# vinits5/learning3d

Measured on AMD Instinct MI355X. Metric: clouds/sec DGCNN-fwd+Chamfer B=32 N=1024; kNN HBM GB/s vs peak at 1/2/4/8 GPU, higher is better.
Workload: dtype f32 (shared-MLP GEMMs as f16x2: fp32 operands carried as an fp16 high part + an fp16 residual (unscaled between the EdgeConv kernel and conv5, 2^12-scaled elsewhere), 3 fp16 MFMA products per fp32 product, f32 accumulate, fp32-level error -- tests bound it by 2x the fp32-MFMA kernel's own error agai

## Files before the change

learning3d_amd/csrc/edgeconv_f16b.hip:

```cpp
#include <type_traits>
#include "common.h"
#include "edgeconv_layout.h"
#include "split_bf16.h"

#define EF_V2 1
#define EF_W4_BYTES ((EC_C4 / 16) * (EC_C3 / 32) * 2 * 1024)
#define EF_PAR_FLOATS (EC5_OFF_SC + 16 - EC5_OFF_W4)
#define EF_PAR_BYTES (EF_PAR_FLOATS * 4)
#define EF_LOFF_B2 (EF_W4_BYTES)
#define EF_LOFF_B3 (EF_LOFF_B2 + 4 * EC_C2)
#define EF_LOFF_B4 (EF_LOFF_B3 + 4 * EC_C3)
#define EF_LOFF_W1 (EF_LOFF_B4 + 4 * EC_C4)
#define EF_LOFF_B1 (EF_LOFF_W1 + 4 * 8 * EC_C1)
#define EF_STG_A (EF_PAR_BYTES)
#define EF_STG_B (EF_STG_A + 4 * 4096)
#define EF_LDS_BYTES (EF_STG_B + 4 * 2048)
static_assert(EC5_OFF_B2 == EC5_OFF_W4 + EF_W4_BYTES / 4 && EC5_OFF_B1 == EC5_OFF_W1 + 8 * EC_C1 && EC5_OFF_SC == EC5_OFF_B1 + EC_C1,
              "the fifth copy's tail is one contiguous run");
static_assert(EF_PAR_BYTES % 16 == 0 && EF_LDS_BYTES <= 163840, "LDS budget");
#define EF_NPL 2
#define EFO_W2 EC5_OFF_W2
#define EFO_W3 EC5_OFF_W3
#define EFO_W4 EC5_OFF_W4
#define EFO_B2 EC5_OFF_B2
#define EFO_B3 EC5_OFF_B3
#define EFO_B4 EC5_OFF_B4
#define EFO_SC EC5_OFF_SC
#define EFO_W1 EC5_OFF_W1
#define EFO_B1 EC5_OFF_B1
#define EF_KERNEL edgeconv_f16b_kernel
#define EF_ENTRY l3d_edgeconv_forward_f16b

typedef _Float16 f16x8 __attribute__((ext_vector_type(8)));
typedef uint32_t u32x4 __attribute__((ext_vector_type(4)));
struct EfBase { const char *p; };
typedef __attribute__((address_space(3))) const char *ef_lds_t;
typedef __attribute__((address_space(3))) const float *ef_ldsf_t;
typedef __attribute__((address_space(3))) char *ef_ldsw_t;
typedef EfBase ef_rsrc_t;

#define EF_ACON "a"
__device__ __forceinline__ void ef_mfma_init(f32x4 &d, const u32x4 &a, const f16x8 &b, const f32x4 &c)
{
    asm volatile("v_mfma_f32_16x16x32_f16 %0, %1, %2, %3" : "=&v"(d) : EF_ACON(a), "a"(b), "v"(c));
}
__device__ __forceinline__ void ef_mfma_acc(f32x4 &d, const u32x4 &a, const f16x8 &b)
{
    asm volatile("v_mfma_f32_16x16x32_f16 %0, %1, %2, %0" : "+v"(d) : EF_ACON(a), "a"(b));
}
__device__ __forceinline__ f16x8 ef_home_agpr(u32x4 v)
{
    f16x8 r = __builtin_bit_cast(f16x8, v);
    asm("" : "+a"(r));
    return r;
}

__device__ __forceinline__ float ef_vmax(float a, float b)
{
    float r;
    asm volatile("v_max_f32 %0, %1, %2" : "=v"(r) : "v"(a), "v"(b));
    return r;
}
__device__ __forceinline__ float ef_vmax3(float a, float b, float c)
{
    float r;
    asm volatile("v_max3_f32 %0, %1, %2, %3" : "=v"(r) : "v"(a), "v"(b), "v"(c));
    return r;
}
__device__ __forceinline__ float ef_dpp_max_x1(float give, float keep)
{
    float r;
    asm volatile("s_nop 1\n\tv_max_f32_dpp %0, %1, %2 quad_perm:[1,0,3,2] row_mask:0xf bank_mask:0xf" : "=v"(r) : "v"(give), "v"(keep));
    return r;
}
__device__ __forceinline__ float ef_dpp_max_x2(float give, float keep)
{
    float r;
    asm volatile("s_nop 1\n\tv_max_f32_dpp %0, %1, %2 quad_perm:[2,3,0,1] row_mask:0xf bank_mask:0xf" : "=v"(r) : "v"(give), "v"(keep));
    return r;
}

__device__ __forceinline__ void ef_split_pair(float a0, float a1, float c, uint32_t &h, uint32_t &m)
{
    (void)c;
    asm volatile("v_cvt_pk_f16_f32 %0, %1, %2" : "=v"(h) : "v"(a0), "v"(a1));
    asm volatile("s_nop 0\n\tv_fma_mixlo_f16 %0, %1, 1.0, -%2 op_sel_hi:[0,0,1]" : "=v"(m) : "v"(a0), "v"(h));
    asm volatile("v_fma_mixhi_f16 %0, %1, 1.0, -%2 op_sel:[0,0,1] op_sel_hi:[0,0,1]" : "+v"(m) : "v"(a1), "v"(h));
}

struct EfLane {
    bool odd, hi;
    unsigned laneoff;
    ef_rsrc_t rs;
    ef_lds_t w4lds;
    float *prow;
    ef_ldsw_t stgA, stgB;
    float mres;
    size_t bn;
};

struct EfScale {
    float split, pool;
};

struct EfTmp {
    f32x4 mx[2];
    u32x4 qh, qm;
    f32x2 xs[2];
};

template <int MT, bool LAST> struct EfN { static constexpr int UNITS = LAST ? 12 : 6 * MT + 12; };

template <int MT, bool LAST, bool RAW, bool PLANES, int U>
__device__ __forceinline__ void ef_micro(f32x4 (&h)[2][MT], f16x8 (&pl)[2][MT], EfTmp &T, int ch0, const EfLane &L, const EfScale &sc, float &ovf)
{
    const float c = sc.split;
    constexpr int NT = LAST ? 0 : 6 * MT;
    if constexpr (U < NT) {
        constexpr int t = U / 6, k = U % 6;
        if constexpr (k < 2) {
#pragma unroll
            for (int r = 0; r < 4; r++) h[k][t][r] = RAW ? ef_vmax(h[k][t][r], 0.f) : fmaxf(h[k][t][r], 0.f);
        } else {
            constexpr int i = k - 2;
            uint32_t a, b;
            ef_split_pair(h[i >> 1][t][2 * (i & 1)], h[i >> 1][t][2 * (i & 1) + 1], c, a, b);
            T.qh[i] = a;
            T.qm[i] = b;
            if constexpr (i == 3) {
                pl[0][t] = ef_home_agpr(T.qh);
                pl[1][t] = ef_home_agpr(T.qm);
            }
        }
    } else if constexpr (U < NT + 8) {
        constexpr int k = (U - NT) / 4, r = (U - NT) % 4;
        static_assert(MT >= 3 && MT <= 5, "row tiles per wave");
        if constexpr (RAW) {
            float m = ef_vmax3(h[k][0][r], h[k][1][r], h[k][2][r]);
            if constexpr (MT == 4) m = ef_vmax(m, h[k][3][r]);
            if constexpr (MT == 5) m = ef_vmax3(m, h[k][3][r], h[k][4][r]);
            T.mx[k][r] = m;
        } else {
            float m = h[k][0][r];
#pragma unroll
            for (int t = 1; t < MT; t++) m = fmaxf(m, h[k][t][r]);
            T.mx[k][r] = m;
        }
    } else {
        constexpr int k = (U - NT - 8) / 2, part = (U - NT - 8) % 2;
        if constexpr (part == 0) {
            const float k0 = L.odd ? T.mx[k][2] : T.mx[k][0], g0 = L.odd ? T.mx[k][0] : T.mx[k][2];
            const float k1 = L.odd ? T.mx[k][3] : T.mx[k][1], g1 = L.odd ? T.mx[k][1] : T.mx[k][3];
            T.xs[k][0] = ef_dpp_max_x1(g0, k0);
            T.xs[k][1] = ef_dpp_max_x1(g1, k1);
        } else {
            const float kk = L.hi ? T.xs[k][1] : T.xs[k][0], gg = L.hi ? T.xs[k][0] : T.xs[k][1];
            float v = ef_dpp_max_x2(gg, kk);
            if constexpr (LAST) v = ef_vmax(v, 0.f);
            if constexpr (!LAST) ovf = ef_vmax(ovf, v * sc.split);
            v *= sc.pool;
            if constexpr (PLANES) {
                ovf = ef_vmax(ovf, v);
                const _Float16 hh = (_Float16)v;
                const _Float16 mm = (_Float16)((v - (float)hh) * L.mres);
                typedef __attribute__((address_space(3))) _Float16 *lh_t;
                if constexpr (!LAST) {
                    const int off = ((ch0 + 16 * k) >> 3) * 64;
                    *(lh_t)(L.stgA + off) = hh;
                    *(lh_t)(L.stgA + off + 2048) = mm;
                } else {
                    const int m = (ch0 - (EC_C1 + EC_C2 + EC_C3)) >> 5;
                    const int off = ((m >> 1) & 1) * 1024 + (m & 1) * 512 + (2 * k) * 64;
                    *(lh_t)(L.stgB + off) = hh;
                    *(lh_t)(L.stgB + off + 256) = mm;
                }
            } else {
                L.prow[ch0 + 16 * k] = v;
            }
        }
    }
}

template <int I0, int I1, class F>
__device__ __forceinline__ void ef_static_for(F &&f)
{
    if constexpr (I0 < I1) {
        f(std::integral_constant<int, I0>{});
        ef_static_for<I0 + 1, I1>(f);
    }
}

template <int MT, bool LAST, bool RAW, bool PLANES>
__device__ __forceinline__ void ef_finish_all(f32x4 (&h)[2][MT], f16x8 (&pl)[2][MT], int ch0, const EfLane &L, const EfScale &sc, float &ovf)
{
    EfTmp T;
    ef_static_for<0, EfN<MT, LAST>::UNITS>([&](auto u) { ef_micro<MT, LAST, RAW, PLANES, decltype(u)::value>(h, pl, T, ch0, L, sc, ovf); });
}

#define EF_PIN() asm volatile("" ::: "memory")

#ifndef EF_PD
#define EF_PD 4
#endif
struct EfRing {
    u32x4 a[EF_PD][EF_NPL];
    f32x4 bv[2];
};
struct EfNext {
    int woff;
    ef_ldsf_t bias;
    int mp;
    int steps;
};

__device__ __forceinline__ u32x4 ef_ldfrag(ef_rsrc_t rs, int byte_off, int frag, unsigned laneoff)
{
    return *(const u32x4 *)(rs.p + (size_t)byte_off + (size_t)frag * 1024 + laneoff);
}

__device__ __forceinline__ u32x4 ef_ldfrag_lds(ef_lds_t base, int frag, unsigned laneoff)
{
    return *(__attribute__((address_space(3))) const u32x4 *)(base + frag * 1024 + laneoff);
}

__device__ __forceinline__ void ef_ring_fill(EfRing &R, ef_rsrc_t rs, int woff, ef_ldsf_t bias4g, int mp, int steps, int lane)
{
#pragma unroll
    for (int d = 0; d < EF_PD; d++)
#pragma unroll
        for (int p = 0; p < EF_NPL; p++) R.a[d][p] = ef_ldfrag(rs, woff, (mp * steps + d) * EF_NPL + p, (unsigned)lane * 16u);
    R.bv[0] = *(__attribute__((address_space(3))) const f32x4 *)(bias4g + 32 * mp);
    R.bv[1] = *(__attribute__((address_space(3))) const f32x4 *)(bias4g + 32 * mp + 16);
}

template <int MT, int S, bool PREV_LAST, bool PREV_RAW, bool PLANES, int NSL, bool OWN_LDS = false, bool NX_LDS = false>
__device__ __forceinline__ void ef_pair(int mp, const EfNext &nx, const f16x8 (&pin)[S][2][MT], const f16x8 (&pin_last)[2][MT],
                                        int woff, EfRing &R,
                                        f32x4 (&acc)[2][MT], f32x4 (&hp)[2][MT], f16x8 (&po_prev)[2][MT],
                                        int ch_prev, const EfLane &L, const EfScale &c_prev, float &ovf)
{
    static_assert(2 * S >= EF_PD, "a pair is at least EF_PD steps long");
    constexpr int NU = EfN<MT, PREV_LAST>::UNITS;
    EfTmp T;
    ef_static_for<0, 2 * S>([&](auto rc) {
        constexpr int r = decltype(rc)::value, s = r >> 1, mm = r & 1;
        u32x4 an[EF_NPL];
        if constexpr (r + EF_PD < 2 * S) {
#pragma unroll
            for (int p = 0; p < EF_NPL; p++)
                an[p] = OWN_LDS ? ef_ldfrag_lds(L.w4lds, (mp * 2 * S + r + EF_PD) * EF_NPL + p, L.laneoff)
                                : ef_ldfrag(L.rs, woff, (mp * 2 * S + r + EF_PD) * EF_NPL + p, L.laneoff);
        } else {
#pragma unroll
            for (int p = 0; p < EF_NPL; p++)
                an[p] = NX_LDS ? ef_ldfrag_lds(L.w4lds, (nx.mp * nx.steps + (r + EF_PD - 2 * S)) * EF_NPL + p, L.laneoff)
                               : ef_ldfrag(L.rs, nx.woff, (nx.mp * nx.steps + (r + EF_PD - 2 * S)) * EF_NPL + p, L.laneoff);
        }
        EF_PIN();
        if constexpr (s == S - 1 && mm == 0 && NSL < 2 * S * 3 * MT)
            asm volatile("s_nop 7");
        ef_static_for<0, 3>([&](auto pc) {
            constexpr int prod = decltype(pc)::value;
            constexpr int pa = prod == 0 ? 1 : 0;
            constexpr int pb = prod == 1 ? 1 : 0;
            ef_static_for<0, MT>([&](auto tc) {
                constexpr int t = decltype(tc)::value;
                const f16x8 &bop = s == S - 1 ? pin_last[pb][t] : pin[s][pb][t];
                if constexpr (s == 0 && prod == 0) ef_mfma_init(acc[mm][t], R.a[0][pa], bop, R.bv[mm]);
                else ef_mfma_acc(acc[mm][t], R.a[0][pa], bop);
                constexpr int slot = (r * 3 + prod) * MT + t;
                if constexpr (slot < NSL)
                    ef_static_for<slot * NU / NSL, (slot + 1) * NU / NSL>([&](auto u) {
                        ef_micro<MT, PREV_LAST, PREV_RAW, PLANES, decltype(u)::value>(hp, po_prev, T, ch_prev, L, c_prev, ovf);
                    });
            });
        });
        if constexpr (r == 1) {
            R.bv[0] = *(__attribute__((address_space(3))) const f32x4 *)(nx.bias + 32 * nx.mp);
            R.bv[1] = *(__attribute__((address_space(3))) const f32x4 *)(nx.bias + 32 * nx.mp + 16);
            EF_PIN();
        }
#pragma unroll
        for (int p = 0; p < EF_NPL; p++) {
#pragma unroll
            for (int d = 0; d + 1 < EF_PD; d++) R.a[d][p] = R.a[d + 1][p];
            R.a[EF_PD - 1][p] = an[p];
        }
    });
}

struct EfNoHook { template <class I> __device__ __forceinline__ void operator()(I) const {} };

template <int MT, int S, int NPAIR, bool LAST, bool UNROLL, bool IN_RAW, bool PLANES, class HOOK = EfNoHook, bool OWN_LDS = false, bool AFTER_LDS = false>
__device__ __forceinline__ void ef_layer(const f16x8 (&pin)[S][2][MT], f16x8 (&pout)[LAST ? 1 : NPAIR][2][MT],
                                         int woff, ef_ldsf_t bias4g, const EfNext &after, EfRing &R, int ch_own,
                                         f32x4 (&accA)[2][MT], f32x4 (&accB)[2][MT], int ch_in,
                                         int *mp_out, const EfLane &L, int rot, const EfScale &c_in, const EfScale &c_own, float &ovf,
                                         HOOK &&hook = EfNoHook())
{
    static_assert(NPAIR % 2 == 0 && S >= 2, "pairs are processed two at a time; deferred finish needs S >= 2");
    constexpr int NS = 2 * S * 3 * MT, NSD = (S - 1) * 6 * MT;
    f16x8 last[2][MT];
    auto in_layer = [&](int mp) { return EfNext{woff, bias4g, mp, 2 * S}; };
    if constexpr (UNROLL) {
        static_assert(NPAIR == 2 || NPAIR == 4, "unrolled layers have 2 or 4 output pairs");
        static_assert(!OWN_LDS, "only the rolled (last) layer keeps its weights in LDS");
        ef_pair<MT, S, false, IN_RAW, PLANES, NSD>(0, in_layer(1), pin, last, woff, R, accA, accB, last, ch_in, L, c_in, ovf);
        if constexpr (NPAIR > 2)
            ef_pair<MT, S, LAST, true, PLANES, NS>(1, in_layer(2), pin, last, woff, R, accB, accA, pout[0], ch_own, L, c_own, ovf);
        else
            ef_pair<MT, S, LAST, true, PLANES, NS, false, AFTER_LDS>(1, after, pin, last, woff, R, accB, accA, pout[0], ch_own, L, c_own, ovf);
        if constexpr (NPAIR == 4) {
            ef_pair<MT, S, LAST, true, PLANES, NS>(2, in_layer(3), pin, last, woff, R, accA, accB, pout[1], ch_own + 32, L, c_own, ovf);
            ef_pair<MT, S, LAST, true, PLANES, NS, false, AFTER_LDS>(3, after, pin, last, woff, R, accB, accA, pout[2], ch_own + 64, L, c_own, ovf);
        }
        *mp_out = NPAIR - 1;
    } else {
        (void)rot;
        ef_pair<MT, S, false, IN_RAW, PLANES, NSD, OWN_LDS, OWN_LDS>(0, in_layer(1), pin, last, woff, R, accA, accB, last, ch_in, L, c_in, ovf);
        ef_static_for<1, NPAIR>([&](auto ic) {
            constexpr int i = decltype(ic)::value;
            hook(ic);
            constexpr bool more = i + 1 < NPAIR;
            const EfNext nx = more ? in_layer(i + 1) : after;
            if constexpr (i & 1)
                ef_pair<MT, S, LAST, true, PLANES, NS, OWN_LDS, more ? OWN_LDS : AFTER_LDS>(i, nx, pin, last, woff, R, accB, accA, pout[0],
                                                                                          ch_own + 32 * (i - 1), L, c_own, ovf);
            else
                ef_pair<MT, S, LAST, true, PLANES, NS, OWN_LDS, more ? OWN_LDS : AFTER_LDS>(i, nx, pin, last, woff, R, accA, accB, pout[0],
                                                                                          ch_own + 32 * (i - 1), L, c_own, ovf);
        });
        *mp_out = NPAIR - 1;
    }
}


template <int MT>
struct EfGather {
    int nb[MT];
    float c;
    float b1[MT];
    int b, nc;
};

template <int MT>
__device__ __forceinline__ void ef_gather_idx(EfGather<MT> &G, int tile, int tiles_per_cloud, int N, int k, const float *__restrict__ xyz,
                                              const int64_t *__restrict__ idx, int wave, int j, int g)
{
    const int b = tile / tiles_per_cloud, xb = tile - b * tiles_per_cloud;
    const int n = (xb * 4 + wave) * 4 + (j >> 2);
    const int nc = min(n, N - 1);
    G.b = b;
    G.nc = nc;
    const float *cloud = xyz + (size_t)b * N * 3;
    G.c = cloud[nc * 3 + (g == 0 ? 1 : 2)];
    const int64_t *row = idx + (size_t)b * N * k;
#pragma unroll
    for (int t = 0; t < MT; t++) {
        const int jj = 4 * t + (j & 3);
        G.nb[t] = (int)row[nc * k + (jj < k ? jj : 0)];
    }
}

template <int MT>
__device__ __forceinline__ void ef_gather_xyz(EfGather<MT> &G, int N, const float *__restrict__ xyz, int g)
{
    const float *cloud = xyz + (size_t)G.b * N * 3;
    const int comp = g < 3 ? g : 0;
#pragma unroll
    for (int t = 0; t < MT; t++) {
        int r = g < 3 ? G.nb[t] : G.nc;
        asm("" : "+v"(r));
        G.b1[t] = cloud[r * 3 + comp];
    }
}

template <int MT, bool PLANES>
__global__ __launch_bounds__(256, 1) void EF_KERNEL(const float *__restrict__ xyz,
                                                              const int64_t *__restrict__ idx, int B, int N, int k,
                                                              const float *packed,
                                                              float *__restrict__ pooled,
                                                              int *__restrict__ range_flag, float mres)
{
#define EF_T(i)
    EF_T(0);
    constexpr int CTOT = EC_C1 + EC_C2 + EC_C3 + EC_C4;
    const int lane = threadIdx.x & 63, wave = threadIdx.x >> 6;
    const int j = lane & 15, g = lane >> 4;
    const int tiles_per_cloud = (N + 15) / 16, ntiles = B * tiles_per_cloud;
    EfLane L;
    L.laneoff = (unsigned)lane * 16u;
    L.rs.p = (const char *)packed;
    L.odd = j & 1;
    L.hi = j & 2;
    const int cl = 4 * g + ((j & 1) * 2 + ((j >> 1) & 1));
    L.bn = (size_t)B * N;
    L.mres = mres;
    extern __shared__ __attribute__((aligned(16))) unsigned char ef_lds[];
    L.w4lds = (ef_lds_t)ef_lds;
    {
        const int cell = (cl >> 3) * 64 + (j >> 2) * 16 + (cl & 7) * 2;
        L.stgA = (ef_ldsw_t)ef_lds + EF_STG_A + wave * 4096 + cell;
        L.stgB = (ef_ldsw_t)ef_lds + EF_STG_B + wave * 2048 + cell;
    }
    typedef __attribute__((address_space(3))) const u32x4 *ef_ldsq_t;
    const ef_ldsq_t rdA = (ef_ldsq_t)((ef_lds_t)ef_lds + EF_STG_A + wave * 4096 + lane * 16);
    const ef_ldsq_t rdB = (ef_ldsq_t)((ef_lds_t)ef_lds + EF_STG_B + wave * 2048 + lane * 16);
    if (PLANES && blockIdx.x == 0 && threadIdx.x == 0)
        *(float *)((_Float16 *)pooled + 2 * 512 * L.bn) = packed[EFO_SC + 12];
    const int po = PLANES ? 8 : 4;
    const EfScale s1 = {packed[EFO_SC + 0], packed[EFO_SC + po + 0]}, s2 = {packed[EFO_SC + 1], packed[EFO_SC + po + 1]},
                  s3 = {packed[EFO_SC + 2], packed[EFO_SC + po + 2]}, s4 = {1.0f, packed[EFO_SC + po + 3]};
    float ovf = 0.f;
    constexpr int w2 = EFO_W2 * 4, w3 = EFO_W3 * 4, w4 = EFO_W4 * 4;
    const ef_ldsf_t bs2 = (ef_ldsf_t)((ef_lds_t)ef_lds + EF_LOFF_B2) + 4 * g, bs3 = (ef_ldsf_t)((ef_lds_t)ef_lds + EF_LOFF_B3) + 4 * g,
                    bs4 = (ef_ldsf_t)((ef_lds_t)ef_lds + EF_LOFF_B4) + 4 * g;

    int tile = blockIdx.x;
    EfGather<MT> G;
    ef_gather_idx<MT>(G, tile, tiles_per_cloud, N, k, xyz, idx, wave, j, g);
    EF_PIN();
    ef_gather_xyz<MT>(G, N, xyz, g);
    EF_PIN();
    {
        typedef const __attribute__((address_space(1))) void *gp_t;
        typedef __attribute__((address_space(3))) void *lp_t;
        constexpr int NCH = EF_PAR_BYTES / 1024;
        const char *src = (const char *)(packed + EFO_W4);
#pragma unroll
        for (int c = 0; c < (NCH + 3) / 4; c++) {
            const int ch = c * 4 + wave;
            if (ch < NCH) __builtin_amdgcn_global_load_lds((gp_t)(src + ch * 1024 + lane * 16), (lp_t)(ef_lds + ch * 1024), 16, 0, 0);
        }
        EF_PIN();
        constexpr int REM = EF_PAR_BYTES - NCH * 1024;
        static_assert(REM % 16 == 0 && REM < 1024, "remainder in 16-byte pieces");
        if (threadIdx.x < REM / 16) ((uint4 *)(ef_lds + NCH * 1024))[threadIdx.x] = ((const uint4 *)(src + NCH * 1024))[threadIdx.x];
    }
    asm volatile("s_waitcnt vmcnt(0)" ::: "memory");
    __syncthreads();
    EfRing R;
    ef_ring_fill(R, L.rs, EFO_W2 * 4, bs2, 0, 2 * (EC_C1 / 32), lane);
    EF_PIN();
#pragma unroll
    for (int t = 0; t < MT; t++) asm volatile("" : "+v"(G.b1[t]));
    asm volatile("" : "+v"(G.c));

    for (; tile < ntiles; tile += gridDim.x) {
    const int b = G.b;
    L.prow = pooled + ((size_t)b * N + G.nc) * CTOT + cl;
    const int n_st = min(((tile - b * tiles_per_cloud) * 4 + wave) * 4 + (lane & 3), N - 1);
    char *const img_pt = (char *)pooled + ((size_t)b * N + n_st) * 16;
    const size_t row_bytes = L.bn * 16;
    float b1[MT][2];
#pragma unroll
    for (int t = 0; t < MT; t++) { b1[t][0] = G.b1[t]; b1[t][1] = g < 2 ? G.c : 0.f; }
    const int tile_next = tile + (int)gridDim.x;
    const bool has_next = tile_next < ntiles;

    EF_T(1);
    f16x8 p1[EC_C1 / 32][2][MT];
    f32x4 accA[2][MT], accB[2][MT];
    {
        typedef __attribute__((address_space(3))) const f32x2 *lw1_t;
        typedef __attribute__((address_space(3))) const f32x4 *lb1_t;
        const lw1_t w1 = (lw1_t)((ef_lds_t)ef_lds + EF_LOFF_W1);
        const ef_ldsf_t b1p = (ef_ldsf_t)((ef_lds_t)ef_lds + EF_LOFF_B1) + 4 * g;
        f32x2 a1[EC_C1 / 16];
        f32x4 bv1[EC_C1 / 16];
#pragma unroll
        for (int m = 0; m < EC_C1 / 16; m++) { a1[m] = w1[m * 64 + lane]; bv1[m] = *(lb1_t)(b1p + 16 * m); }
        static_assert(EC_C1 == 64, "layer 1 is two M-tile pairs");
        auto mfma1 = [&](f32x4 &d, float a, float b, const f32x4 &c, bool first) {
            if (first) asm volatile("v_mfma_f32_16x16x4_f32 %0, %1, %2, %3" : "=&v"(d) : "v"(a), "v"(b), "v"(c));
            else asm volatile("v_mfma_f32_16x16x4_f32 %0, %1, %2, %0" : "+v"(d) : "v"(a), "v"(b));
        };
#pragma unroll
        for (int t = 0; t < MT; t++) asm volatile("" ::"v"(b1[t][0]), "v"(b1[t][1]));
        asm volatile("s_nop 3");
#pragma unroll
        for (int mm = 0; mm < 2; mm++)
#pragma unroll
            for (int s = 0; s < 2; s++)
#pragma unroll
                for (int t = 0; t < MT; t++) mfma1(accA[mm][t], a1[mm][s], b1[t][s], bv1[mm], s == 0);
        constexpr int NU1 = EfN<MT, false>::UNITS, NSL1 = 4 * MT;
        EfTmp T1;
        ef_static_for<0, NSL1>([&](auto sc) {
            constexpr int slot = decltype(sc)::value, mm = slot / (2 * MT), s = (slot / MT) % 2, t = slot % MT;
            mfma1(accB[mm][t], a1[2 + mm][s], b1[t][s], bv1[2 + mm], s == 0);
            ef_static_for<slot * NU1 / NSL1, (slot + 1) * NU1 / NSL1>([&](auto u) {
                ef_micro<MT, false, true, PLANES, decltype(u)::value>(accA, p1[0], T1, 0, L, s1, ovf);
            });
        });
#pragma unroll
        for (int m = 0; m < EC_C1 / 16; m++) asm volatile("" ::"v"(bv1[m]), "v"(a1[m]));
    }
    int mp_last;

    EF_T(2);
    f16x8 p2[EC_C2 / 32][2][MT];
    ef_layer<MT, EC_C1 / 32, EC_C2 / 32, false, true, true, PLANES>(
        p1, p2, w2, bs2, EfNext{w3, bs3, 0, 2 * (EC_C2 / 32)}, R, EC_C1, accA, accB,
        32 * (EC_C1 / 32 - 1), &mp_last, L, 0, s1, s2, ovf);
    EF_T(3);
    f16x8 p3[EC_C3 / 32][2][MT];
    ef_layer<MT, EC_C2 / 32, EC_C3 / 32, false, true, true, PLANES, EfNoHook, false, true>(
        p2, p3, w3, bs3, EfNext{w4, bs4, 0, 2 * (EC_C3 / 32)}, R, EC_C1 + EC_C2, accA, accB,
        EC_C1 + 32 * (EC_C2 / 32 - 1), &mp_last, L, 0, s2, s3, ovf);
    EF_T(4);
    f16x8 dummy[1][2][MT];
    u32x4 X;
#define EF_ST16(ptr, val) (*(u32x4 *)(ptr) = (val))
    auto st_a = [&](int c) { EF_ST16(img_pt + (size_t)((c >> 1) * 64 + (c & 1) * 16 + (lane >> 2)) * row_bytes, X); EF_PIN(); };
    auto st_b = [&](int m0) {
        const int row = ((lane >> 4) & 1) * 64 + (EC_C1 + EC_C2 + EC_C3) / 8 + 4 * (m0 + (lane >> 5)) + ((lane >> 2) & 3);
        EF_ST16(img_pt + (size_t)row * row_bytes, X);
        EF_PIN();
    };
    auto hook = [&](auto ic) {
        constexpr int i = decltype(ic)::value;
        if constexpr (PLANES) {
            if constexpr (i >= 2 && i <= 5) st_a(i - 2);
            if constexpr (i == 6) st_b(0);
            if constexpr (i == 7) st_b(2);
            if constexpr (i >= 1 && i <= 4) X = rdA[(i - 1) * 64];
            if constexpr (i == 5 || i == 7) X = rdB[0];
            if constexpr (i == 6) X = rdB[64];
            EF_PIN();
        }
        if (has_next) {
            if constexpr (i == 2) { ef_gather_idx<MT>(G, tile_next, tiles_per_cloud, N, k, xyz, idx, wave, j, g); EF_PIN(); }
            if constexpr (i == 6) { ef_gather_xyz<MT>(G, N, xyz, g); EF_PIN(); }
            if constexpr (i == 7) {
#pragma unroll
                for (int t = 0; t < MT; t++) asm volatile("" : "+v"(G.b1[t]));
                asm volatile("" : "+v"(G.c));
            }
        }
    };
    ef_layer<MT, EC_C3 / 32, EC_C4 / 32, true, false, true, PLANES, decltype(hook) &, true, false>(
        p3, dummy, w4, bs4, EfNext{w2, bs2, 0, 2 * (EC_C1 / 32)}, R, EC_C1 + EC_C2 + EC_C3, accA, accB,
        EC_C1 + EC_C2 + 32 * (EC_C3 / 32 - 1), &mp_last, L, 0, s3, s4, ovf, hook);
    if constexpr (PLANES) st_b(4);
    asm volatile("s_nop 15\n\ts_nop 15");
    ef_finish_all<MT, true, true, PLANES>(accB, dummy[0], EC_C1 + EC_C2 + EC_C3 + 32 * mp_last, L, s4, ovf);
    if constexpr (PLANES) { X = rdB[64]; st_b(6); }
    EF_T(5);
    }
    if (!(ovf <= 60000.f) && range_flag) *(volatile int *)range_flag = 1;
}

static int ef_grid(int ntiles)
{
    static thread_local int cus[16] = {0};
    int dev = 0;
    if (hipGetDevice(&dev) != hipSuccess || dev < 0 || dev >= 16) dev = 0;
    if (cus[dev] == 0) {
        int n = 0;
        if (hipDeviceGetAttribute(&n, hipDeviceAttributeMultiprocessorCount, dev) != hipSuccess || n <= 0) n = 256;
        cus[dev] = n;
    }
    return ntiles < cus[dev] ? ntiles : cus[dev];
}

extern "C" int EF_ENTRY(const float *xyz, const int64_t *idx, int B, int N, int k,
                                        const float *packed, void *out, int out_mode, int *range_flag, l3d_stream_t stream)
{
    L3D_REQUIRE(xyz && idx && packed && out && B > 0 && N > 0 && k > 0 && out_mode >= 0 && out_mode <= 2);
    const float mres = out_mode == 2 ? 1.0f : 4096.0f;
    if (k > 20 || B > 65535 || (((size_t)packed) & 15) || (((size_t)out) & 15)) return L3D_ERR_UNSUPPORTED;
    const long ntiles = (long)B * l3d_divup(N, 16);
    if (ntiles > 0x7fffffffL / 2) return L3D_ERR_UNSUPPORTED;
    dim3 grid(ef_grid((int)ntiles)), block(256);
    hipStream_t st = (hipStream_t)stream;
    float *o = (float *)out;
    const size_t lds = EF_LDS_BYTES;
    if (out_mode == 0) {
        if (k <= 16) hipLaunchKernelGGL((EF_KERNEL<4, false>), grid, block, lds, st, xyz, idx, B, N, k, packed, o, range_flag, mres);
        else              hipLaunchKernelGGL((EF_KERNEL<5, false>), grid, block, lds, st, xyz, idx, B, N, k, packed, o, range_flag, mres);
    } else {
        if (k <= 16) hipLaunchKernelGGL((EF_KERNEL<4, true>), grid, block, lds, st, xyz, idx, B, N, k, packed, o, range_flag, mres);
        else              hipLaunchKernelGGL((EF_KERNEL<5, true>), grid, block, lds, st, xyz, idx, B, N, k, packed, o, range_flag, mres);
    }
    return l3d_check_launch();
}
```

Before: 118,100.

## Defer pooled-channel plane split into later layer and rebalance epilogue interleave

Pooled max results for the first three layers are now kept in AGPRs and converted to fp16 hi/residual planes later, during the last layer's MFMA steps, through a staged unpark hook. Before this, the split and LDS stores ran right after each layer. The quad-reduction and split helpers are merged into multi-instruction asm blocks that use SGPR lane masks with v_cndmask instead of per-lane bools. Epilogue micro-units are now spread over MFMA slots by weighted cost rather than uniformly. The aim is to hide VALU epilogue work under matrix ops. The cost is higher AGPR pressure and a fragile compile-time schedule.

```diff
diff --git a/learning3d_amd/csrc/edgeconv_f16b.hip b/learning3d_amd/csrc/edgeconv_f16b.hip
--- a/learning3d_amd/csrc/edgeconv_f16b.hip
+++ b/learning3d_amd/csrc/edgeconv_f16b.hip
@@ -61,35 +61,87 @@
     asm volatile("v_max_f32 %0, %1, %2" : "=v"(r) : "v"(a), "v"(b));
     return r;
 }
-__device__ __forceinline__ float ef_vmax3(float a, float b, float c)
+
+template <int MT>
+__device__ __forceinline__ float ef_pool_rows(float a0, float a1, float a2, float a3, float a4)
 {
     float r;
-    asm volatile("v_max3_f32 %0, %1, %2, %3" : "=v"(r) : "v"(a), "v"(b), "v"(c));
+    if constexpr (MT == 3) asm volatile("v_max3_f32 %0, %1, %2, %3" : "=v"(r) : "v"(a0), "v"(a1), "v"(a2));
+    if constexpr (MT == 4) asm volatile("v_max3_f32 %0, %1, %2, %3\n\tv_max_f32 %0, %0, %4" : "=&v"(r) : "v"(a0), "v"(a1), "v"(a2), "v"(a3));
+    if constexpr (MT == 5)
+        asm volatile("v_max3_f32 %0, %1, %2, %3\n\tv_max3_f32 %0, %0, %4, %5" : "=&v"(r) : "v"(a0), "v"(a1), "v"(a2), "v"(a3), "v"(a4));
     return r;
 }
-__device__ __forceinline__ float ef_dpp_max_x1(float give, float keep)
-{
-    float r;
-    asm volatile("s_nop 1\n\tv_max_f32_dpp %0, %1, %2 quad_perm:[1,0,3,2] row_mask:0xf bank_mask:0xf" : "=v"(r) : "v"(give), "v"(keep));
-    return r;
-}
-__device__ __forceinline__ float ef_dpp_max_x2(float give, float keep)
-{
-    float r;
-    asm volatile("s_nop 1\n\tv_max_f32_dpp %0, %1, %2 quad_perm:[2,3,0,1] row_mask:0xf bank_mask:0xf" : "=v"(r) : "v"(give), "v"(keep));
-    return r;
-}
-
-__device__ __forceinline__ void ef_split_pair(float a0, float a1, float c, uint32_t &h, uint32_t &m)
-{
-    (void)c;
-    asm volatile("v_cvt_pk_f16_f32 %0, %1, %2" : "=v"(h) : "v"(a0), "v"(a1));
-    asm volatile("s_nop 0\n\tv_fma_mixlo_f16 %0, %1, 1.0, -%2 op_sel_hi:[0,0,1]" : "=v"(m) : "v"(a0), "v"(h));
-    asm volatile("v_fma_mixhi_f16 %0, %1, 1.0, -%2 op_sel:[0,0,1] op_sel_hi:[0,0,1]" : "+v"(m) : "v"(a1), "v"(h));
+
+__device__ __forceinline__ void ef_quad_step1(const f32x4 &a, const f32x4 &b, uint64_t odd, f32x2 &xa, f32x2 &xb)
+{
+    float k0, g0, k1, g1, k2, g2, k3, g3, r0, r1, r2, r3;
+    asm volatile("v_cndmask_b32 %[k0], %[a0], %[a2], %[odd]\n\t"
+                 "v_cndmask_b32 %[g0], %[a2], %[a0], %[odd]\n\t"
+                 "v_cndmask_b32 %[k1], %[a1], %[a3], %[odd]\n\t"
+                 "v_cndmask_b32 %[g1], %[a3], %[a1], %[odd]\n\t"
+                 "v_cndmask_b32 %[k2], %[b0], %[b2], %[odd]\n\t"
+                 "v_cndmask_b32 %[g2], %[b2], %[b0], %[odd]\n\t"
+                 "v_cndmask_b32 %[k3], %[b1], %[b3], %[odd]\n\t"
+                 "v_cndmask_b32 %[g3], %[b3], %[b1], %[odd]\n\t"
+                 "v_max_f32_dpp %[r0], %[g0], %[k0] quad_perm:[1,0,3,2] row_mask:0xf bank_mask:0xf\n\t"
+                 "v_max_f32_dpp %[r1], %[g1], %[k1] quad_perm:[1,0,3,2] row_mask:0xf bank_mask:0xf\n\t"
+                 "v_max_f32_dpp %[r2], %[g2], %[k2] quad_perm:[1,0,3,2] row_mask:0xf bank_mask:0xf\n\t"
+                 "v_max_f32_dpp %[r3], %[g3], %[k3] quad_perm:[1,0,3,2] row_mask:0xf bank_mask:0xf"
+                 : [k0] "=&v"(k0), [g0] "=&v"(g0), [k1] "=&v"(k1), [g1] "=&v"(g1), [k2] "=&v"(k2), [g2] "=&v"(g2), [k3] "=&v"(k3),
+                   [g3] "=&v"(g3), [r0] "=&v"(r0), [r1] "=&v"(r1), [r2] "=&v"(r2), [r3] "=&v"(r3)
+                 : [a0] "v"(a[0]), [a1] "v"(a[1]), [a2] "v"(a[2]), [a3] "v"(a[3]), [b0] "v"(b[0]), [b1] "v"(b[1]), [b2] "v"(b[2]),
+                   [b3] "v"(b[3]), [odd] "s"(odd));
+    xa[0] = r0; xa[1] = r1; xb[0] = r2; xb[1] = r3;
+}
+
+template <bool LAST>
+__device__ __forceinline__ void ef_quad_step2(const f32x2 &xa, const f32x2 &xb, uint64_t hi, float split, float &va, float &vb, float &ovf)
+{
+    float k0, g0, k1, g1, t0, t1;
+    if constexpr (LAST) {
+        (void)split; (void)t0; (void)t1; (void)ovf;
+        asm volatile("v_cndmask_b32 %[k0], %[a0], %[a1], %[hi]\n\t"
+                     "v_cndmask_b32 %[g0], %[a1], %[a0], %[hi]\n\t"
+                     "v_cndmask_b32 %[k1], %[b0], %[b1], %[hi]\n\t"
+                     "v_cndmask_b32 %[g1], %[b1], %[b0], %[hi]\n\t"
+                     "v_max_f32_dpp %[va], %[g0], %[k0] quad_perm:[2,3,0,1] row_mask:0xf bank_mask:0xf\n\t"
+                     "v_max_f32_e64 %[va], %[va], 0\n\t"
+                     "v_max_f32_dpp %[vb], %[g1], %[k1] quad_perm:[2,3,0,1] row_mask:0xf bank_mask:0xf\n\t"
+                     "v_max_f32_e64 %[vb], %[vb], 0"
+                     : [k0] "=&v"(k0), [g0] "=&v"(g0), [k1] "=&v"(k1), [g1] "=&v"(g1), [va] "=&v"(va), [vb] "=&v"(vb)
+                     : [a0] "v"(xa[0]), [a1] "v"(xa[1]), [b0] "v"(xb[0]), [b1] "v"(xb[1]), [hi] "s"(hi));
+    } else {
+        asm volatile("v_cndmask_b32 %[k0], %[a0], %[a1], %[hi]\n\t"
+                     "v_cndmask_b32 %[g0], %[a1], %[a0], %[hi]\n\t"
+                     "v_cndmask_b32 %[k1], %[b0], %[b1], %[hi]\n\t"
+                     "v_cndmask_b32 %[g1], %[b1], %[b0], %[hi]\n\t"
+                     "v_max_f32_dpp %[va], %[g0], %[k0] quad_perm:[2,3,0,1] row_mask:0xf bank_mask:0xf\n\t"
+                     "v_mul_f32 %[t0], %[va], %[sp]\n\t"
+                     "v_max_f32_dpp %[vb], %[g1], %[k1] quad_perm:[2,3,0,1] row_mask:0xf bank_mask:0xf\n\t"
+                     "v_mul_f32 %[t1], %[vb], %[sp]\n\t"
+                     "v_max_f32 %[ovf], %[ovf], %[t0]\n\t"
+                     "v_max_f32 %[ovf], %[ovf], %[t1]"
+                     : [k0] "=&v"(k0), [g0] "=&v"(g0), [k1] "=&v"(k1), [g1] "=&v"(g1), [va] "=&v"(va), [vb] "=&v"(vb), [t0] "=&v"(t0),
+                       [t1] "=&v"(t1), [ovf] "+v"(ovf)
+                     : [a0] "v"(xa[0]), [a1] "v"(xa[1]), [b0] "v"(xb[0]), [b1] "v"(xb[1]), [hi] "s"(hi), [sp] "v"(split));
+    }
+}
+
+__device__ __forceinline__ void ef_split_2pairs(float a0, float a1, float b0, float b1, uint32_t &ha, uint32_t &ma, uint32_t &hb, uint32_t &mb)
+{
+    asm volatile("v_cvt_pk_f16_f32 %0, %4, %5\n\t"
+                 "v_cvt_pk_f16_f32 %2, %6, %7\n\t"
+                 "v_fma_mixlo_f16 %1, %4, 1.0, -%0 op_sel_hi:[0,0,1]\n\t"
+                 "v_fma_mixlo_f16 %3, %6, 1.0, -%2 op_sel_hi:[0,0,1]\n\t"
+                 "v_fma_mixhi_f16 %1, %5, 1.0, -%0 op_sel:[0,0,1] op_sel_hi:[0,0,1]\n\t"
+                 "v_fma_mixhi_f16 %3, %7, 1.0, -%2 op_sel:[0,0,1] op_sel_hi:[0,0,1]"
+                 : "=&v"(ha), "=&v"(ma), "=&v"(hb), "=&v"(mb)
+                 : "v"(a0), "v"(a1), "v"(b0), "v"(b1));
 }
 
 struct EfLane {
-    bool odd, hi;
+    uint64_t odd, hi;
     unsigned laneoff;
     ef_rsrc_t rs;
     ef_lds_t w4lds;
@@ -103,31 +155,71 @@
     float split, pool;
 };
 
+struct EfOut {
+    float ovf;
+    float park[(EC_C1 + EC_C2 + EC_C3) / 16];
+    float last[2];
+};
+
+struct EfStage {
+    float v, t;
+    uint32_t h, m;
+};
+template <int G, bool PARKED>
+__device__ __forceinline__ void ef_unpark(EfStage &s, float parked, float pool, float mres, float &ovf, ef_ldsw_t cell)
+{
+    typedef __attribute__((address_space(3))) _Float16 *lh_t;
+    if constexpr (G == 0 && PARKED) asm volatile("v_accvgpr_read_b32 %0, %1\n\tv_mul_f32 %0, %2, %0" : "=&v"(s.v) : "a"(parked), "s"(pool));
+    if constexpr (G == 0 && !PARKED) asm volatile("v_mul_f32 %0, %2, %1" : "=v"(s.v) : "v"(parked), "s"(pool));
+    if constexpr (G == 1) asm volatile("v_max_f32 %0, %0, %2\n\tv_cvt_f16_f32 %1, %2" : "+v"(ovf), "=&v"(s.h) : "v"(s.v));
+    if constexpr (G == 2) asm volatile("v_cvt_f32_f16 %0, %1\n\tv_sub_f32 %0, %2, %0" : "=&v"(s.t) : "v"(s.h), "v"(s.v));
+    if constexpr (G == 3) asm volatile("v_mul_f32 %0, %2, %1\n\tv_cvt_f16_f32 %0, %0" : "=&v"(s.m) : "v"(s.t), "s"(mres));
+    if constexpr (G == 4) {
+        *(lh_t)cell = __builtin_bit_cast(_Float16, (uint16_t)s.h);
+        *(lh_t)(cell + (PARKED ? 2048 : 256)) = __builtin_bit_cast(_Float16, (uint16_t)s.m);
+    }
+}
+
 struct EfTmp {
     f32x4 mx[2];
     u32x4 qh, qm;
     f32x2 xs[2];
 };
 
-template <int MT, bool LAST> struct EfN { static constexpr int UNITS = LAST ? 12 : 6 * MT + 12; };
+template <int MT, bool LAST> struct EfN {
+    static constexpr int NT = LAST ? 0 : 6 * MT;
+    static constexpr int UNITS = NT + 10;
+    static constexpr int weight(int u) { return u < NT ? (u % 6 < 4 ? 2 : 8) : u < NT + 8 ? 2 : u == NT + 8 ? 12 : LAST ? 20 : 12; }
+    static constexpr int first(int u0, int u1, int n, int s)
+    {
+        int W = 0, cum = 0;
+        for (int u = u0; u < u1; u++) W += weight(u);
+        for (int u = u0; u < u1; u++) {
+            if (cum * n / W >= s) return u;
+            cum += weight(u);
+        }
+        return u1;
+    }
+};
 
 template <int MT, bool LAST, bool RAW, bool PLANES, int U>
-__device__ __forceinline__ void ef_micro(f32x4 (&h)[2][MT], f16x8 (&pl)[2][MT], EfTmp &T, int ch0, const EfLane &L, const EfScale &sc, float &ovf)
-{
-    const float c = sc.split;
-    constexpr int NT = LAST ? 0 : 6 * MT;
+__device__ __forceinline__ void ef_micro(f32x4 (&h)[2][MT], f16x8 (&pl)[2][MT], EfTmp &T, int ch0, const EfLane &L, const EfScale &sc, EfOut &O)
+{
+    constexpr int NT = EfN<MT, LAST>::NT;
     if constexpr (U < NT) {
         constexpr int t = U / 6, k = U % 6;
-        if constexpr (k < 2) {
-#pragma unroll
-            for (int r = 0; r < 4; r++) h[k][t][r] = RAW ? ef_vmax(h[k][t][r], 0.f) : fmaxf(h[k][t][r], 0.f);
+        if constexpr (k < 4) {
+#pragma unroll
+            for (int r = 2 * (k & 1); r < 2 * (k & 1) + 2; r++) h[k >> 1][t][r] = RAW ? ef_vmax(h[k >> 1][t][r], 0.f) : fmaxf(h[k >> 1][t][r], 0.f);
         } else {
-            constexpr int i = k - 2;
-            uint32_t a, b;
-            ef_split_pair(h[i >> 1][t][2 * (i & 1)], h[i >> 1][t][2 * (i & 1) + 1], c, a, b);
-            T.qh[i] = a;
-            T.qm[i] = b;
-            if constexpr (i == 3) {
+            constexpr int m = k - 4;
+            uint32_t ha, ma, hb, mb;
+            ef_split_2pairs(h[m][t][0], h[m][t][1], h[m][t][2], h[m][t][3], ha, ma, hb, mb);
+            T.qh[2 * m] = ha;
+            T.qm[2 * m] = ma;
+            T.qh[2 * m + 1] = hb;
+            T.qm[2 * m + 1] = mb;
+            if constexpr (m == 1) {
                 pl[0][t] = ef_home_agpr(T.qh);
                 pl[1][t] = ef_home_agpr(T.qm);
             }
@@ -136,46 +228,28 @@
         constexpr int k = (U - NT) / 4, r = (U - NT) % 4;
         static_assert(MT >= 3 && MT <= 5, "row tiles per wave");
         if constexpr (RAW) {
-            float m = ef_vmax3(h[k][0][r], h[k][1][r], h[k][2][r]);
-            if constexpr (MT == 4) m = ef_vmax(m, h[k][3][r]);
-            if constexpr (MT == 5) m = ef_vmax3(m, h[k][3][r], h[k][4][r]);
-            T.mx[k][r] = m;
+            T.mx[k][r] = ef_pool_rows<MT>(h[k][0][r], h[k][1][r], h[k][2][r], h[k][MT > 3 ? 3 : 0][r], h[k][MT > 4 ? 4 : 0][r]);
         } else {
             float m = h[k][0][r];
 #pragma unroll
             for (int t = 1; t < MT; t++) m = fmaxf(m, h[k][t][r]);
             T.mx[k][r] = m;
         }
+    } else if constexpr (U == NT + 8) {
+        ef_quad_step1(T.mx[0], T.mx[1], L.odd, T.xs[0], T.xs[1]);
     } else {
-        constexpr int k = (U - NT - 8) / 2, part = (U - NT - 8) % 2;
-        if constexpr (part == 0) {
-            const float k0 = L.odd ? T.mx[k][2] : T.mx[k][0], g0 = L.odd ? T.mx[k][0] : T.mx[k][2];
-            const float k1 = L.odd ? T.mx[k][3] : T.mx[k][1], g1 = L.odd ? T.mx[k][1] : T.mx[k][3];
-            T.xs[k][0] = ef_dpp_max_x1(g0, k0);
-            T.xs[k][1] = ef_dpp_max_x1(g1, k1);
-        } else {
-            const float kk = L.hi ? T.xs[k][1] : T.xs[k][0], gg = L.hi ? T.xs[k][0] : T.xs[k][1];
-            float v = ef_dpp_max_x2(gg, kk);
-            if constexpr (LAST) v = ef_vmax(v, 0.f);
-            if constexpr (!LAST) ovf = ef_vmax(ovf, v * sc.split);
-            v *= sc.pool;
-            if constexpr (PLANES) {
-                ovf = ef_vmax(ovf, v);
-                const _Float16 hh = (_Float16)v;
-                const _Float16 mm = (_Float16)((v - (float)hh) * L.mres);
-                typedef __attribute__((address_space(3))) _Float16 *lh_t;
-                if constexpr (!LAST) {
-                    const int off = ((ch0 + 16 * k) >> 3) * 64;
-                    *(lh_t)(L.stgA + off) = hh;
-                    *(lh_t)(L.stgA + off + 2048) = mm;
-                } else {
-                    const int m = (ch0 - (EC_C1 + EC_C2 + EC_C3)) >> 5;
-                    const int off = ((m >> 1) & 1) * 1024 + (m & 1) * 512 + (2 * k) * 64;
-                    *(lh_t)(L.stgB + off) = hh;
-                    *(lh_t)(L.stgB + off + 256) = mm;
-                }
+        float vk[2];
+        ef_quad_step2<LAST>(T.xs[0], T.xs[1], L.hi, sc.split, vk[0], vk[1], O.ovf);
+#pragma unroll
+        for (int k = 0; k < 2; k++) {
+            if constexpr (PLANES && !LAST) {
+                float p = vk[k];
+                asm("" : "+a"(p));
+                O.park[(ch0 >> 4) + k] = p;
+            } else if constexpr (PLANES) {
+                O.last[k] = vk[k];
             } else {
-                L.prow[ch0 + 16 * k] = v;
+                L.prow[ch0 + 16 * k] = vk[k] * sc.pool;
             }
         }
     }
@@ -190,11 +264,25 @@
     }
 }
 
+template <int G>
+__device__ __forceinline__ void ef_last_stage(EfStage &s, EfOut &O, int k, int ch0, const EfLane &L, const EfScale &sc)
+{
+    const int m = (ch0 - (EC_C1 + EC_C2 + EC_C3)) >> 5;
+    ef_unpark<G, false>(s, O.last[k], sc.pool, L.mres, O.ovf, L.stgB + ((m >> 1) & 1) * 1024 + (m & 1) * 512 + (2 * k) * 64);
+}
+
 template <int MT, bool LAST, bool RAW, bool PLANES>
-__device__ __forceinline__ void ef_finish_all(f32x4 (&h)[2][MT], f16x8 (&pl)[2][MT], int ch0, const EfLane &L, const EfScale &sc, float &ovf)
+__device__ __forceinline__ void ef_finish_all(f32x4 (&h)[2][MT], f16x8 (&pl)[2][MT], int ch0, const EfLane &L, const EfScale &sc, EfOut &O)
 {
     EfTmp T;
-    ef_static_for<0, EfN<MT, LAST>::UNITS>([&](auto u) { ef_micro<MT, LAST, RAW, PLANES, decltype(u)::value>(h, pl, T, ch0, L, sc, ovf); });
+    ef_static_for<0, EfN<MT, LAST>::UNITS>([&](auto u) { ef_micro<MT, LAST, RAW, PLANES, decltype(u)::value>(h, pl, T, ch0, L, sc, O); });
+    if constexpr (LAST && PLANES) {
+        EfStage s[2];
+        ef_static_for<0, 5>([&](auto g) {
+            ef_last_stage<decltype(g)::value>(s[0], O, 0, ch0, L, sc);
+            ef_last_stage<decltype(g)::value>(s[1], O, 1, ch0, L, sc);
+        });
+    }
 }
 
 #define EF_PIN() asm volatile("" ::: "memory")
@@ -233,14 +321,23 @@
     R.bv[1] = *(__attribute__((address_space(3))) const f32x4 *)(bias4g + 32 * mp + 16);
 }
 
-template <int MT, int S, bool PREV_LAST, bool PREV_RAW, bool PLANES, int NSL, bool OWN_LDS = false, bool NX_LDS = false>
+struct EfNoHook { template <class... I> __device__ __forceinline__ void operator()(I...) const {} };
+
+template <int MT, int S, bool PREV_LAST, bool PREV_RAW, bool PLANES, int NSL, bool OWN_LDS = false, bool NX_LDS = false, class EXTRA = EfNoHook>
 __device__ __forceinline__ void ef_pair(int mp, const EfNext &nx, const f16x8 (&pin)[S][2][MT], const f16x8 (&pin_last)[2][MT],
                                         int woff, EfRing &R,
                                         f32x4 (&acc)[2][MT], f32x4 (&hp)[2][MT], f16x8 (&po_prev)[2][MT],
-                                        int ch_prev, const EfLane &L, const EfScale &c_prev, float &ovf)
+                                        int ch_prev, const EfLane &L, const EfScale &c_prev, EfOut &O, EXTRA &&extra = EfNoHook())
 {
     static_assert(2 * S >= EF_PD, "a pair is at least EF_PD steps long");
-    constexpr int NU = EfN<MT, PREV_LAST>::UNITS;
+    typedef EfN<MT, PREV_LAST> E;
+    constexpr int NU = E::UNITS, NS = 2 * S * 3 * MT;
+    constexpr int NA = NSL < NS ? E::NT : NU;
+    constexpr bool WAYOUT = PREV_LAST && PLANES;
+    constexpr int NSU = WAYOUT ? (2 * S - 5) * 3 * MT : NSL;
+    static_assert(!WAYOUT || (2 * S > 5 && NSL == NS), "five steps for the way out");
+    EfStage TS[2];
+    static_assert(NSL == NS || !PREV_LAST, "a deferred finish is the finish of a layer that has planes");
     EfTmp T;
     ef_static_for<0, 2 * S>([&](auto rc) {
         constexpr int r = decltype(rc)::value, s = r >> 1, mm = r & 1;
@@ -269,10 +366,14 @@
                 if constexpr (s == 0 && prod == 0) ef_mfma_init(acc[mm][t], R.a[0][pa], bop, R.bv[mm]);
                 else ef_mfma_acc(acc[mm][t], R.a[0][pa], bop);
                 constexpr int slot = (r * 3 + prod) * MT + t;
-                if constexpr (slot < NSL)
-                    ef_static_for<slot * NU / NSL, (slot + 1) * NU / NSL>([&](auto u) {
-                        ef_micro<MT, PREV_LAST, PREV_RAW, PLANES, decltype(u)::value>(hp, po_prev, T, ch_prev, L, c_prev, ovf);
-                    });
+                constexpr int ub = slot < NSU ? E::first(0, NA, NSU, slot) : WAYOUT ? NU : E::first(NA, NU, NS - NSL, slot - NSL);
+                constexpr int ue = slot < NSU ? E::first(0, NA, NSU, slot + 1) : WAYOUT ? NU : E::first(NA, NU, NS - NSL, slot + 1 - NSL);
+                ef_static_for<ub, ue>([&](auto u) {
+                    ef_micro<MT, PREV_LAST, PREV_RAW, PLANES, decltype(u)::value>(hp, po_prev, T, ch_prev, L, c_prev, O);
+                });
+                if constexpr (WAYOUT && slot >= NSU && (slot % (3 * MT) == 5 || slot % (3 * MT) == 10))
+                    ef_last_stage<(slot - NSU) / (3 * MT)>(TS[slot % (3 * MT) == 10], O, slot % (3 * MT) == 10, ch_prev, L, c_prev);
+                extra(std::integral_constant<int, slot>{});
             });
         });
         if constexpr (r == 1) {
@@ -289,14 +390,14 @@
     });
 }
 
-struct EfNoHook { template <class I> __device__ __forceinline__ void operator()(I) const {} };
-
-template <int MT, int S, int NPAIR, bool LAST, bool UNROLL, bool IN_RAW, bool PLANES, class HOOK = EfNoHook, bool OWN_LDS = false, bool AFTER_LDS = false>
+
+template <int MT, int S, int NPAIR, bool LAST, bool UNROLL, bool IN_RAW, bool PLANES, class HOOK = EfNoHook, bool OWN_LDS = false, bool AFTER_LDS = false,
+          class EXTRA = EfNoHook>
 __device__ __forceinline__ void ef_layer(const f16x8 (&pin)[S][2][MT], f16x8 (&pout)[LAST ? 1 : NPAIR][2][MT],
                                          int woff, ef_ldsf_t bias4g, const EfNext &after, EfRing &R, int ch_own,
                                          f32x4 (&accA)[2][MT], f32x4 (&accB)[2][MT], int ch_in,
-                                         int *mp_out, const EfLane &L, int rot, const EfScale &c_in, const EfScale &c_own, float &ovf,
-                                         HOOK &&hook = EfNoHook())
+                                         int *mp_out, const EfLane &L, int rot, const EfScale &c_in, const EfScale &c_own, EfOut &O,
+                                         HOOK &&hook = EfNoHook(), EXTRA &&extra = EfNoHook())
 {
     static_assert(NPAIR % 2 == 0 && S >= 2, "pairs are processed two at a time; deferred finish needs S >= 2");
     constexpr int NS = 2 * S * 3 * MT, NSD = (S - 1) * 6 * MT;
@@ -305,30 +406,31 @@
     if constexpr (UNROLL) {
         static_assert(NPAIR == 2 || NPAIR == 4, "unrolled layers have 2 or 4 output pairs");
         static_assert(!OWN_LDS, "only the rolled (last) layer keeps its weights in LDS");
-        ef_pair<MT, S, false, IN_RAW, PLANES, NSD>(0, in_layer(1), pin, last, woff, R, accA, accB, last, ch_in, L, c_in, ovf);
+        ef_pair<MT, S, false, IN_RAW, PLANES, NSD>(0, in_layer(1), pin, last, woff, R, accA, accB, last, ch_in, L, c_in, O);
         if constexpr (NPAIR > 2)
-            ef_pair<MT, S, LAST, true, PLANES, NS>(1, in_layer(2), pin, last, woff, R, accB, accA, pout[0], ch_own, L, c_own, ovf);
+            ef_pair<MT, S, LAST, true, PLANES, NS>(1, in_layer(2), pin, last, woff, R, accB, accA, pout[0], ch_own, L, c_own, O);
         else
-            ef_pair<MT, S, LAST, true, PLANES, NS, false, AFTER_LDS>(1, after, pin, last, woff, R, accB, accA, pout[0], ch_own, L, c_own, ovf);
+            ef_pair<MT, S, LAST, true, PLANES, NS, false, AFTER_LDS>(1, after, pin, last, woff, R, accB, accA, pout[0], ch_own, L, c_own, O);
         if constexpr (NPAIR == 4) {
-            ef_pair<MT, S, LAST, true, PLANES, NS>(2, in_layer(3), pin, last, woff, R, accA, accB, pout[1], ch_own + 32, L, c_own, ovf);
-            ef_pair<MT, S, LAST, true, PLANES, NS, false, AFTER_LDS>(3, after, pin, last, woff, R, accB, accA, pout[2], ch_own + 64, L, c_own, ovf);
+            ef_pair<MT, S, LAST, true, PLANES, NS>(2, in_layer(3), pin, last, woff, R, accA, accB, pout[1], ch_own + 32, L, c_own, O);
+            ef_pair<MT, S, LAST, true, PLANES, NS, false, AFTER_LDS>(3, after, pin, last, woff, R, accB, accA, pout[2], ch_own + 64, L, c_own, O);
         }
         *mp_out = NPAIR - 1;
     } else {
         (void)rot;
-        ef_pair<MT, S, false, IN_RAW, PLANES, NSD, OWN_LDS, OWN_LDS>(0, in_layer(1), pin, last, woff, R, accA, accB, last, ch_in, L, c_in, ovf);
+        ef_pair<MT, S, false, IN_RAW, PLANES, NSD, OWN_LDS, OWN_LDS>(0, in_layer(1), pin, last, woff, R, accA, accB, last, ch_in, L, c_in, O);
         ef_static_for<1, NPAIR>([&](auto ic) {
             constexpr int i = decltype(ic)::value;
             hook(ic);
             constexpr bool more = i + 1 < NPAIR;
             const EfNext nx = more ? in_layer(i + 1) : after;
+            auto ex = [&](auto sc) { extra(ic, sc); };
             if constexpr (i & 1)
-                ef_pair<MT, S, LAST, true, PLANES, NS, OWN_LDS, more ? OWN_LDS : AFTER_LDS>(i, nx, pin, last, woff, R, accB, accA, pout[0],
-                                                                                          ch_own + 32 * (i - 1), L, c_own, ovf);
+                ef_pair<MT, S, LAST, true, PLANES, NS, OWN_LDS, more ? OWN_LDS : AFTER_LDS, decltype(ex) &>(i, nx, pin, last, woff, R, accB, accA, pout[0],
+                                                                                                           ch_own + 32 * (i - 1), L, c_own, O, ex);
             else
-                ef_pair<MT, S, LAST, true, PLANES, NS, OWN_LDS, more ? OWN_LDS : AFTER_LDS>(i, nx, pin, last, woff, R, accA, accB, pout[0],
-                                                                                          ch_own + 32 * (i - 1), L, c_own, ovf);
+                ef_pair<MT, S, LAST, true, PLANES, NS, OWN_LDS, more ? OWN_LDS : AFTER_LDS, decltype(ex) &>(i, nx, pin, last, woff, R, accA, accB, pout[0],
+                                                                                                           ch_own + 32 * (i - 1), L, c_own, O, ex);
         });
         *mp_out = NPAIR - 1;
     }
@@ -391,8 +493,8 @@
     EfLane L;
     L.laneoff = (unsigned)lane * 16u;
     L.rs.p = (const char *)packed;
-    L.odd = j & 1;
-    L.hi = j & 2;
+    L.odd = __ballot(j & 1);
+    L.hi = __ballot(j & 2);
     const int cl = 4 * g + ((j & 1) * 2 + ((j >> 1) & 1));
     L.bn = (size_t)B * N;
     L.mres = mres;
@@ -411,7 +513,8 @@
     const int po = PLANES ? 8 : 4;
     const EfScale s1 = {packed[EFO_SC + 0], packed[EFO_SC + po + 0]}, s2 = {packed[EFO_SC + 1], packed[EFO_SC + po + 1]},
                   s3 = {packed[EFO_SC + 2], packed[EFO_SC + po + 2]}, s4 = {1.0f, packed[EFO_SC + po + 3]};
-    float ovf = 0.f;
+    EfOut O;
+    O.ovf = 0.f;
     constexpr int w2 = EFO_W2 * 4, w3 = EFO_W3 * 4, w4 = EFO_W4 * 4;
     const ef_ldsf_t bs2 = (ef_ldsf_t)((ef_lds_t)ef_lds + EF_LOFF_B2) + 4 * g, bs3 = (ef_ldsf_t)((ef_lds_t)ef_lds + EF_LOFF_B3) + 4 * g,
                     bs4 = (ef_ldsf_t)((ef_lds_t)ef_lds + EF_LOFF_B4) + 4 * g;
@@ -489,8 +592,8 @@
         ef_static_for<0, NSL1>([&](auto sc) {
             constexpr int slot = decltype(sc)::value, mm = slot / (2 * MT), s = (slot / MT) % 2, t = slot % MT;
             mfma1(accB[mm][t], a1[2 + mm][s], b1[t][s], bv1[2 + mm], s == 0);
-            ef_static_for<slot * NU1 / NSL1, (slot + 1) * NU1 / NSL1>([&](auto u) {
-                ef_micro<MT, false, true, PLANES, decltype(u)::value>(accA, p1[0], T1, 0, L, s1, ovf);
+            ef_static_for<EfN<MT, false>::first(0, NU1, NSL1, slot), EfN<MT, false>::first(0, NU1, NSL1, slot + 1)>([&](auto u) {
+                ef_micro<MT, false, true, PLANES, decltype(u)::value>(accA, p1[0], T1, 0, L, s1, O);
             });
         });
 #pragma unroll
@@ -502,17 +605,17 @@
     f16x8 p2[EC_C2 / 32][2][MT];
     ef_layer<MT, EC_C1 / 32, EC_C2 / 32, false, true, true, PLANES>(
         p1, p2, w2, bs2, EfNext{w3, bs3, 0, 2 * (EC_C2 / 32)}, R, EC_C1, accA, accB,
-        32 * (EC_C1 / 32 - 1), &mp_last, L, 0, s1, s2, ovf);
+        32 * (EC_C1 / 32 - 1), &mp_last, L, 0, s1, s2, O);
     EF_T(3);
     f16x8 p3[EC_C3 / 32][2][MT];
     ef_layer<MT, EC_C2 / 32, EC_C3 / 32, false, true, true, PLANES, EfNoHook, false, true>(
         p2, p3, w3, bs3, EfNext{w4, bs4, 0, 2 * (EC_C3 / 32)}, R, EC_C1 + EC_C2, accA, accB,
-        EC_C1 + 32 * (EC_C2 / 32 - 1), &mp_last, L, 0, s2, s3, ovf);
+        EC_C1 + 32 * (EC_C2 / 32 - 1), &mp_last, L, 0, s2, s3, O);
     EF_T(4);
     f16x8 dummy[1][2][MT];
-    u32x4 X;
+    u32x4 X, XA;
 #define EF_ST16(ptr, val) (*(u32x4 *)(ptr) = (val))
-    auto st_a = [&](int c) { EF_ST16(img_pt + (size_t)((c >> 1) * 64 + (c & 1) * 16 + (lane >> 2)) * row_bytes, X); EF_PIN(); };
+    auto st_a = [&](int c) { EF_ST16(img_pt + (size_t)((c >> 1) * 64 + (c & 1) * 16 + (lane >> 2)) * row_bytes, XA); EF_PIN(); };
     auto st_b = [&](int m0) {
         const int row = ((lane >> 4) & 1) * 64 + (EC_C1 + EC_C2 + EC_C3) / 8 + 4 * (m0 + (lane >> 5)) + ((lane >> 2) & 3);
         EF_ST16(img_pt + (size_t)row * row_bytes, X);
@@ -521,10 +624,10 @@
     auto hook = [&](auto ic) {
         constexpr int i = decltype(ic)::value;
         if constexpr (PLANES) {
-            if constexpr (i >= 2 && i <= 5) st_a(i - 2);
+            if constexpr (i >= 4) st_a(i - 4);
             if constexpr (i == 6) st_b(0);
             if constexpr (i == 7) st_b(2);
-            if constexpr (i >= 1 && i <= 4) X = rdA[(i - 1) * 64];
+            if constexpr (i >= 3 && i <= 6) XA = rdA[(i - 3) * 64];
             if constexpr (i == 5 || i == 7) X = rdB[0];
             if constexpr (i == 6) X = rdB[64];
             EF_PIN();
@@ -539,16 +642,31 @@
             }
         }
     };
-    ef_layer<MT, EC_C3 / 32, EC_C4 / 32, true, false, true, PLANES, decltype(hook) &, true, false>(
+    EfStage stg[(EC_C1 + EC_C2 + EC_C3) / 16];
+    auto unpark = [&](auto ic, auto sc) {
+        constexpr int i = decltype(ic)::value, slot = decltype(sc)::value;
+        if constexpr (PLANES && (i == 1 || i == 2)) {
+            constexpr int step = (i - 1) * 2 * (EC_C3 / 32) + slot / (3 * MT), pos = slot % (3 * MT);
+            static_assert(3 * MT >= 12, "ten stage slots and two of ef_pair's in a step");
+            constexpr int pi = pos == 1 ? 0 : pos == 2 ? 1 : pos == 3 ? 2 : pos == 4 ? 3 : pos == 6 ? 4
+                             : pos == 7 ? 5 : pos == 8 ? 6 : pos == 9 ? 7 : pos == 11 ? 8 : pos == 0 ? 9 : -1;
+            if constexpr (pi >= 0) {
+                constexpr int g = pi % 5, e = step - g, w = 2 * e + pi / 5;
+                if constexpr (e >= 0 && e < (EC_C1 + EC_C2 + EC_C3) / 32)
+                    ef_unpark<g, true>(stg[w], O.park[w], w < 4 ? s1.pool : w < 8 ? s2.pool : s3.pool, L.mres, O.ovf, L.stgA + 128 * w);
+            }
+        }
+    };
+    ef_layer<MT, EC_C3 / 32, EC_C4 / 32, true, false, true, PLANES, decltype(hook) &, true, false, decltype(unpark) &>(
         p3, dummy, w4, bs4, EfNext{w2, bs2, 0, 2 * (EC_C1 / 32)}, R, EC_C1 + EC_C2 + EC_C3, accA, accB,
-        EC_C1 + EC_C2 + 32 * (EC_C3 / 32 - 1), &mp_last, L, 0, s3, s4, ovf, hook);
+        EC_C1 + EC_C2 + 32 * (EC_C3 / 32 - 1), &mp_last, L, 0, s3, s4, O, hook, unpark);
     if constexpr (PLANES) st_b(4);
     asm volatile("s_nop 15\n\ts_nop 15");
-    ef_finish_all<MT, true, true, PLANES>(accB, dummy[0], EC_C1 + EC_C2 + EC_C3 + 32 * mp_last, L, s4, ovf);
+    ef_finish_all<MT, true, true, PLANES>(accB, dummy[0], EC_C1 + EC_C2 + EC_C3 + 32 * mp_last, L, s4, O);
     if constexpr (PLANES) { X = rdB[64]; st_b(6); }
     EF_T(5);
     }
-    if (!(ovf <= 60000.f) && range_flag) *(volatile int *)range_flag = 1;
+    if (!(O.ovf <= 60000.f) && range_flag) *(volatile int *)range_flag = 1;
 }
 
 static int ef_grid(int ntiles)
```

Result: faster. 122,300, median of 6 (+3.6%).
